# ChenyangLEI/All-In-One-Deflicker

Measured on NVIDIA H100. Metric: atlas_iters_per_sec, higher is better.
Workload: dtype fp32 (2-term fp16 split on wgmma, fp32 accumulate)

## Files before the change

### all-in-one-deflicker_b200/csrc/mlp_tc.cu

```cuda
#include <mutex>
#include <vector>

#include "tc_api.cuh"
#include "tc_ptx.cuh"
#include "loss_math.h"

namespace b200 {
using namespace ptx;

constexpr int TM = 128;
constexpr int HID = 256;
constexpr int ITEM_BYTES = 16384;
constexpr int CHUNK_BYTES = 4 * ITEM_BYTES;
constexpr float S_ACT = 16.0f;
constexpr float S_W = 256.0f;
constexpr int ATOM_BYTES = TM * 128;
constexpr int TILE_IMG_BYTES = 4 * ATOM_BYTES;
constexpr int PE_COLS = 40;

__host__ __device__ __forceinline__ int atom_off(int m, int k) {
  const int r = m & 7;
  return (m >> 3) * 1024 + r * 128 + (((k >> 3) ^ r) << 4) + ((k & 7) << 1);
}
__host__ __device__ __forceinline__ int item_off(int n, int k) {
  return (n >> 3) * 512 + (n & 7) * 64 + ((((k >> 3) ^ (n >> 1)) & 3) << 4) + ((k & 7) << 1);
}

struct NetImages {
  char* w_fwd; int64_t w_fwd_layer[B200_MAX_LAYERS]; int n_chunks_fwd[B200_MAX_LAYERS];
  char* w_bwd; int64_t w_bwd_layer[B200_MAX_LAYERS];
  char* act; char* dz;
  int64_t slot_stride, term_stride;
  char* pe; char* dzl; int64_t w64_term_stride;
  uint32_t* bits;
  int64_t rows;
};

struct TcLayout { NetImages map, atl; };

static char* align_tc(char* base) { return reinterpret_cast<char*>(round_up(reinterpret_cast<int64_t>(base), 1024)); }
static char* carve_tc(char*& p, int64_t bytes) { char* r = p; p += round_up(bytes, 1024); return r; }

static void plan_fwd_weights(const MlpShape& s, TcNet net, char*& p, NetImages* n) {
  const bool pe = tc_pe_first(net);
  int64_t off = 0;
  for (int l = 0; l < s.L; ++l) {
    int chunks = 0;
    const bool tc_layer = pe ? (l <= s.L - 2) : (l >= 1 && l <= s.L - 2);
    if (tc_layer) chunks = (l == 0 ? 0 : HID / 64) + ((l == 0 || s.skip[l]) && pe ? 1 : 0);
    n->n_chunks_fwd[l] = chunks;
    n->w_fwd_layer[l] = off;
    off += (int64_t)chunks * CHUNK_BYTES;
  }
  n->w_fwd = carve_tc(p, off);
}

static void plan_net(const MlpShape& s, int64_t rows, TcNet net, char*& p, NetImages* n) {
  const int64_t tiles = rows / TM;
  const bool pe = tc_pe_first(net);
  n->rows = rows;
  plan_fwd_weights(s, net, p, n);
  int64_t off = 0;
  for (int l = 0; l < s.L; ++l) {
    n->w_bwd_layer[l] = off;
    const bool used = l <= s.L - 2 && (pe || l >= 1);
    if (used) off += (int64_t)(HID / 64) * CHUNK_BYTES;
  }
  n->w_bwd = carve_tc(p, off);
  n->term_stride = tiles * TILE_IMG_BYTES;
  n->slot_stride = 2 * n->term_stride;
  n->act = carve_tc(p, (int64_t)(s.L - 1) * n->slot_stride);
  n->dz = carve_tc(p, (int64_t)(s.L - 1) * n->slot_stride);
  n->w64_term_stride = tiles * ATOM_BYTES;
  n->pe = pe ? carve_tc(p, 2 * n->w64_term_stride) : nullptr;
  n->dzl = carve_tc(p, 2 * n->w64_term_stride);
  n->bits = reinterpret_cast<uint32_t*>(carve_tc(p, (int64_t)(s.L - 1) * rows * 32));
}

int64_t tc_plan(const MlpShape& ms, const MlpShape& as, int64_t rows_map, int64_t rows_atlas, char* base,
                TcPlan* out) {
  char* p = align_tc(base);
  TcLayout lay{};
  plan_net(ms, rows_map, tc_net_of(ms), p, &lay.map);
  plan_net(as, rows_atlas, TcNet::Atlas, p, &lay.atl);
  if (out) { out->base = base; out->bytes = p - base; out->rows_map = rows_map; out->rows_atlas = rows_atlas; }
  return p - base;
}

static TcLayout layout_of(const TcStep& s) {
  char* p = align_tc(s.plan->base);
  TcLayout lay{};
  plan_net(*s.ms, s.plan->rows_map, tc_net_of(*s.ms), p, &lay.map);
  plan_net(*s.as, s.plan->rows_atlas, TcNet::Atlas, p, &lay.atl);
  return lay;
}

struct PrepJob {
  const float* W; int ldw;
  int n_rows, k0, k_cnt;
  int transpose;
  char* hi; char* lo;
};
constexpr int MAX_PREP_JOBS = 96;
struct PrepJobs { PrepJob j[MAX_PREP_JOBS]; int n; };

__global__ void tc_prep_kernel(const PrepJobs* __restrict__ jobs_ptr) {
  const PrepJob jb = jobs_ptr->j[blockIdx.x >> 2];
  for (int e = threadIdx.x; e < 64 * 8; e += blockDim.x) {
    const int row = (blockIdx.x & 3) * 64 + (e >> 3), c8 = (e & 7) * 8;
    float v[8];
#pragma unroll
    for (int q = 0; q < 8; ++q) {
      const int col = c8 + q;
      v[q] = 0.f;
      if (row < jb.n_rows && col < jb.k_cnt)
        v[q] = jb.transpose ? jb.W[(int64_t)(jb.k0 + col) * jb.ldw + row] : jb.W[(int64_t)row * jb.ldw + jb.k0 + col];
    }
    uint32_t h[4], l[4];
#pragma unroll
    for (int q = 0; q < 4; ++q) split2_f16(v[2 * q] * S_W, v[2 * q + 1] * S_W, h[q], l[q]);
    const int off = (c8 >> 5) * ITEM_BYTES + item_off(row, c8 & 31);
    *reinterpret_cast<uint4*>(jb.hi + off) = make_uint4(h[0], h[1], h[2], h[3]);
    *reinterpret_cast<uint4*>(jb.lo + off) = make_uint4(l[0], l[1], l[2], l[3]);
  }
}

template <int NST>
struct Pipe {
  uint64_t* full; uint64_t* empty; char* stage;
  uint32_t it;
  __device__ __forceinline__ int slot() const { return it % NST; }
  __device__ __forceinline__ uint32_t parity() const { return (it / NST) & 1; }
};

struct TileIter {
  int t0, tf, tb, total, cap_tiles, n_groups, gf, gb;
  __device__ __forceinline__ void init(int cap, int groups, const int* counters, int g_fwd, int g_bwd) {
    cap_tiles = cap / TM;
    n_groups = groups;
    gf = (counters && g_fwd < groups) ? g_fwd : -1;
    gb = (counters && g_bwd < groups) ? g_bwd : -1;
    t0 = counters ? min(cap_tiles, (counters[0] + TM - 1) / TM) : cap_tiles;
    tf = gf >= 0 ? min(cap_tiles, (counters[5] + TM - 1) / TM) : t0;
    tb = gb >= 0 ? min(cap_tiles, (counters[6] + TM - 1) / TM) : t0;
    total = t0 * (groups - (gf >= 0) - (gb >= 0)) + (gf >= 0 ? tf : 0) + (gb >= 0 ? tb : 0);
  }
  __device__ __forceinline__ int group_tiles(int g) const { return g == gf ? tf : (g == gb ? tb : t0); }
  __device__ __forceinline__ int global_tile(int t) const {
    for (int g = 0; g < n_groups; ++g) {
      const int n = group_tiles(g);
      if (t < n) return g * cap_tiles + t;
      t -= n;
    }
    return 0;
  }
};

template <int NST>
__device__ __forceinline__ void produce_items(Pipe<NST>& pp, const char* src, int n_items, uint32_t bytes = ITEM_BYTES) {
  for (int i = 0; i < n_items; ++i) {
    mbar_wait(&pp.empty[pp.slot()], pp.parity() ^ 1);
    mbar_expect_tx(&pp.full[pp.slot()], bytes);
    bulk_g2s(pp.stage + pp.slot() * ITEM_BYTES, src + (int64_t)i * ITEM_BYTES, bytes, &pp.full[pp.slot()]);
    ++pp.it;
  }
}

constexpr int CONSUMER_WGS = 2;
constexpr int CONSUMERS = CONSUMER_WGS * 128;
constexpr int TC_THREADS = CONSUMERS + 128;
constexpr int PRODUCER_REGS = 56, CONSUMER_REGS = 224;
constexpr int EMPTY_ARRIVALS = CONSUMER_WGS * 4;
constexpr int WG_ROW_BYTES = 8192;

struct Consumer {
  int g, w4, lane, q, tid;
  int m0;
  bool warp_leader, leader;
  __device__ __forceinline__ void init() {
    const int warp = warp_uniform();
    lane = threadIdx.x & 31; q = lane & 3;
    g = warp >> 2; w4 = warp & 3;
    tid = threadIdx.x & 127;
    m0 = 64 * g + 16 * w4 + (lane >> 2);
    warp_leader = lane == 0;
    leader = tid == 0;
  }
  __device__ __forceinline__ void sync() const { named_bar(1 + g, 128); }
};

__host__ __device__ __forceinline__ int tile_off(int m, int col) { return (col >> 6) * ATOM_BYTES + atom_off(m, col & 63); }

template <int NST, int NN>
__device__ __forceinline__ void consume_item(Pipe<NST>& pp, float (&acc)[NN / 2], uint32_t a_hi, uint32_t a_lo, bool with_lo,
                                             uint32_t& scale, int& pending, const Consumer& c) {
  mbar_wait(&pp.full[pp.slot()], pp.parity());
  const uint32_t sb = smem_u32(pp.stage + pp.slot() * ITEM_BYTES);
  wgmma_fence();
#pragma unroll
  for (int ks = 0; ks < 2; ++ks) {
    const uint64_t bd = make_desc_sw64(sb + ks * 32, 512);
    if constexpr (NN == 256) wgmma_n256<0, 0>(*reinterpret_cast<float(*)[128]>(&acc), make_desc(a_hi + ks * 32, 16, 1024), bd, scale);
    else wgmma_n64<0, 0>(*reinterpret_cast<float(*)[32]>(&acc), make_desc(a_hi + ks * 32, 16, 1024), bd, scale);
    scale = 1u;
    if (with_lo) {
      if constexpr (NN == 256) wgmma_n256<0, 0>(*reinterpret_cast<float(*)[128]>(&acc), make_desc(a_lo + ks * 32, 16, 1024), bd, 1u);
      else wgmma_n64<0, 0>(*reinterpret_cast<float(*)[32]>(&acc), make_desc(a_lo + ks * 32, 16, 1024), bd, 1u);
    }
  }
  wgmma_commit();
  wgmma_wait<1>();
  if (pending >= 0 && c.warp_leader) mbar_arrive(&pp.empty[pending]);
  pending = pp.slot();
  ++pp.it;
}
template <int NST, int NN>
__device__ __forceinline__ void consume_chunk(Pipe<NST>& pp, float (&acc)[NN / 2], uint32_t a_hi, uint32_t a_lo,
                                              uint32_t& scale, int& pending, const Consumer& c) {
  consume_item<NST, NN>(pp, acc, a_hi, a_lo, true, scale, pending, c);
  consume_item<NST, NN>(pp, acc, a_hi + 64, a_lo + 64, true, scale, pending, c);
  consume_item<NST, NN>(pp, acc, a_hi, a_lo, false, scale, pending, c);
  consume_item<NST, NN>(pp, acc, a_hi + 64, a_lo + 64, false, scale, pending, c);
}
template <int NST, int R>
__device__ __forceinline__ void finish_pass(Pipe<NST>& pp, float (&acc)[R], int& pending, const Consumer& c) {
  wgmma_wait<0>();
  acc_fence(acc);
  if (pending >= 0 && c.warp_leader) mbar_arrive(&pp.empty[pending]);
  pending = -1;
}

__device__ __forceinline__ void store_tile_rows(const Consumer& c, const char* a_tile, char* g_img, int64_t term_stride) {
  if (!c.leader) return;
#pragma unroll
  for (int term = 0; term < 2; ++term)
#pragma unroll
    for (int j = 0; j < 4; ++j)
      bulk_s2g(g_img + term * term_stride + j * ATOM_BYTES + c.g * WG_ROW_BYTES,
               a_tile + term * TILE_IMG_BYTES + j * ATOM_BYTES + c.g * WG_ROW_BYTES, WG_ROW_BYTES);
  bulk_commit();
}
__device__ __forceinline__ void a_tile_reusable(const Consumer& c) {
  if (c.leader) bulk_wait_read0();
  c.sync();
}
__device__ __forceinline__ void a_tile_written(const Consumer& c) {
  fence_proxy_async_smem();
  c.sync();
}

__device__ __forceinline__ uint32_t relu_flag(float v) { return (uint32_t)(-(int)__float_as_uint(v)) >> 31; }

__device__ __forceinline__ uint32_t piece_bits(uint32_t f0, uint32_t f1, int col) {
  const int i = col & 15;
  uint32_t b = (f0 << (15 - i)) | (f1 << (14 - i));
  return b;
}
__device__ __forceinline__ uint32_t quad_or(uint32_t b) {
  b |= __shfl_xor_sync(0xffffffffu, b, 1);
  b |= __shfl_xor_sync(0xffffffffu, b, 2);
  return b;
}
__device__ __forceinline__ float quad_sum(float v) {
  v += __shfl_xor_sync(0xffffffffu, v, 1);
  return v + __shfl_xor_sync(0xffffffffu, v, 2);
}

constexpr int SMEM_A = 2 * TILE_IMG_BYTES;
constexpr int SMEM_AUX = 2 * ATOM_BYTES;
constexpr int RSUM_B_BYTES = 64 * 16;
constexpr int BWD_ACC_FLOATS = 5 * 256 + 768;
constexpr int SMEM_BWD_CONST_FLOATS = CONSUMER_WGS * (RSUM_B_BYTES / 4 + BWD_ACC_FLOATS);
constexpr int SMEM_BARS = 256;
constexpr int SMEM_MAX = 227 * 1024;
template <bool ATLAS, bool BWD> struct KCfg {
  static constexpr int NST = BWD ? 5 : (ATLAS ? 4 : 6);
  static constexpr int SMEM = SMEM_A + NST * ITEM_BYTES + (ATLAS && !BWD ? SMEM_AUX : 0) +
                              (BWD ? SMEM_BWD_CONST_FLOATS * 4 : 0) + SMEM_BARS;
  static_assert(SMEM <= SMEM_MAX, "fused kernel exceeds the shared memory of one CTA");
  static_assert(SMEM + ITEM_BYTES > SMEM_MAX, "one more weight slot would fit");
  static_assert(2 * NST * 8 <= SMEM_BARS, "ring barriers exceed their shared-memory slot");
};

template <int NST>
struct SmemMap {
  char* a_tile; char* stage; char* aux; float* cst;
  uint64_t* full; uint64_t* empty;
  __device__ __forceinline__ void init(char* raw, int aux_bytes, int cst_floats) {
    char* p = raw;
    a_tile = p; p += SMEM_A;
    stage = p; p += NST * ITEM_BYTES;
    aux = p; p += aux_bytes;
    cst = reinterpret_cast<float*>(p); p += cst_floats * 4;
    full = reinterpret_cast<uint64_t*>(p);
    empty = full + NST;
  }
};

template <int NST>
__device__ __forceinline__ void setup_cta(SmemMap<NST>& sm) {
  if (threadIdx.x == 0) {
    if (smem_u32(sm.a_tile) & 1023u) __trap();
    for (int i = 0; i < NST; ++i) { mbar_init(&sm.full[i], 1); mbar_init(&sm.empty[i], EMPTY_ARRIVALS); }
    fence_barrier_init();
  }
  __syncthreads();
}
constexpr int BAR_CONSUMERS = 9;

struct FwdParams {
  const float* x;
  float* y;
  const float* params;
  int64_t w_off[B200_MAX_LAYERS], b_off[B200_MAX_LAYERS];
  NetImages img;
  int cap, n_groups; const int* n_valid;
  int g_fwd, g_bwd;
  float in_scale, in_shift;
  int store_images;
  int tanh_out;
  int pe_freqs;
};

template <bool ATLAS, int NL = (ATLAS ? 8 : 6), int VAR = 0>
__global__ void __launch_bounds__(TC_THREADS, 1) tc_fwd_kernel(const __grid_constant__ FwdParams P) {
  extern __shared__ __align__(1024) char smem_raw[];
  constexpr int NST = KCfg<ATLAS, false>::NST;
  SmemMap<NST> sm; sm.init(smem_raw, ATLAS ? SMEM_AUX : 0, 0);
  const int warp = warp_uniform(), lane = threadIdx.x & 31;
  constexpr int L = NL;
  constexpr int FIRST_TC = ATLAS ? 0 : 1;
  constexpr int LAST_TC = L - 2;
  constexpr bool PE3 = ATLAS && VAR > 0;
  constexpr bool SKIPS = ATLAS && !PE3;
  constexpr int OUT = ATLAS ? (PE3 ? VAR : 3) : 2;
  constexpr int KLAST = SKIPS ? 296 : 256;
  const int pe_cols = VAR == 1 ? 30 : 6 * P.pe_freqs;
  setup_cta(sm);
  TileIter ti; ti.init(P.cap, P.n_groups, P.n_valid, P.g_fwd, P.g_bwd);

  if (warp >= CONSUMER_WGS * 4) {
    setmaxnreg_dec<PRODUCER_REGS>();
    if (warp == CONSUMER_WGS * 4 && lane == 0) {
      Pipe<NST> pp{sm.full, sm.empty, sm.stage, 0};
      for (int t = blockIdx.x; t < ti.total; t += gridDim.x)
        for (int l = FIRST_TC; l <= LAST_TC; ++l) {
          const char* base = P.img.w_fwd + P.img.w_fwd_layer[l];
          if (ATLAS && l == 0) { produce_items(pp, base, 4); continue; }
          if (SKIPS && l == 4) produce_items(pp, base + (int64_t)4 * CHUNK_BYTES, 4);
          produce_items(pp, base, 16);
        }
    }
    return;
  }
  setmaxnreg_inc<CONSUMER_REGS>();
  Consumer c; c.init();
  Pipe<NST> pp{sm.full, sm.empty, sm.stage, 0};
  int pending = -1;
  const float inv_scale = 1.0f / S_W;
  uint16_t* bits16 = reinterpret_cast<uint16_t*>(P.img.bits);
  const float* wlast = P.params + P.w_off[L - 1];
  const uint32_t a_rows = smem_u32(sm.a_tile) + c.g * WG_ROW_BYTES;
  const uint32_t aux_rows = smem_u32(sm.aux) + c.g * WG_ROW_BYTES;
  float acc[128];
  for (int t = blockIdx.x; t < ti.total; t += gridDim.x) {
    const int gt = ti.global_tile(t);
    const int64_t row0 = (int64_t)gt * TM + c.m0;
    auto put = [&](int m, int col, float v0, float v1) {
      uint32_t h, lo;
      split2_packed(v0, v1, h, lo);
      const int off = tile_off(m, col);
      *reinterpret_cast<uint32_t*>(sm.a_tile + off) = h;
      *reinterpret_cast<uint32_t*>(sm.a_tile + TILE_IMG_BYTES + off) = lo;
    };
    uint32_t held0 = 0, held1 = 0;
    auto flags_out = [&](int slot, int i, int col, uint32_t b0, uint32_t b1) {
      if ((i & 1) == 0) { held0 = b0; held1 = b1; return; }
      b0 = quad_or(b0 | held0); b1 = quad_or(b1 | held1);
      if (P.store_images && c.q == 0) {
        bits16[((int64_t)slot * P.img.rows + row0) * 16 + (col >> 4)] = (uint16_t)b0;
        bits16[((int64_t)slot * P.img.rows + row0 + 8) * 16 + (col >> 4)] = (uint16_t)b1;
      }
    };
    if (ATLAS) {
      c.sync();
      for (int task = c.tid; task < 64 * 8; task += 128) {
        const int m = 64 * c.g + (task & 63), c8 = task >> 6;
        const int64_t row = (int64_t)gt * TM + m;
        float in[3] = {0.f, 0.f, 0.f};
        if (PE3) {
          const float4 xv = *reinterpret_cast<const float4*>(P.x + row * 4);
          in[0] = xv.x * P.in_scale + P.in_shift; in[1] = xv.y * P.in_scale + P.in_shift; in[2] = xv.z * P.in_scale + P.in_shift;
        } else {
          const float2 uv = *reinterpret_cast<const float2*>(P.x + row * 2);
          in[0] = uv.x * P.in_scale + P.in_shift; in[1] = uv.y * P.in_scale + P.in_shift;
        }
        float vals[8];
        if (PE3) {
#pragma unroll
          for (int i = 0; i < 8; ++i) {
            const int cc = c8 * 8 + i;
            float v = 0.f;
            if (cc < pe_cols) {
              const int k = cc / 6, r = cc - k * 6;
              const float a = in[r < 3 ? r : r - 3] * pe_freq(k);
              v = r < 3 ? sinf(a) : cosf(a);
            }
            vals[i] = v * S_ACT;
          }
        } else {
#pragma unroll
          for (int half_k = 0; half_k < 2; ++half_k) {
            const int k = c8 * 2 + half_k;
            float s0 = 0.f, s1 = 0.f, c0 = 0.f, c1 = 0.f;
            if (k < 10) {
              const float bk = pe_freq(k);
              const float a0 = in[0] * bk, a1 = in[1] * bk;
              s0 = sinf(a0); s1 = sinf(a1); c0 = cosf(a0); c1 = cosf(a1);
            }
            vals[half_k * 4 + 0] = s0 * S_ACT; vals[half_k * 4 + 1] = s1 * S_ACT;
            vals[half_k * 4 + 2] = c0 * S_ACT; vals[half_k * 4 + 3] = c1 * S_ACT;
          }
        }
        uint32_t h[4], lo[4];
#pragma unroll
        for (int q2 = 0; q2 < 4; ++q2) split2_f16(vals[2 * q2], vals[2 * q2 + 1], h[q2], lo[q2]);
        const int off = atom_off(m, c8 * 8);
        const uint4 vh = make_uint4(h[0], h[1], h[2], h[3]), vl = make_uint4(lo[0], lo[1], lo[2], lo[3]);
        *reinterpret_cast<uint4*>(sm.aux + off) = vh;
        *reinterpret_cast<uint4*>(sm.aux + ATOM_BYTES + off) = vl;
        if (P.store_images) {
          char* g_hi = P.img.pe + (int64_t)gt * ATOM_BYTES;
          *reinterpret_cast<uint4*>(g_hi + off) = vh;
          *reinterpret_cast<uint4*>(g_hi + P.img.w64_term_stride + off) = vl;
        }
      }
      fence_proxy_async_smem();
      c.sync();
    } else {
      const float4 x0 = *reinterpret_cast<const float4*>(P.x + row0 * 4);
      const float4 x1 = *reinterpret_cast<const float4*>(P.x + (row0 + 8) * 4);
      const float* W0 = P.params + P.w_off[0];
      const float* b0p = P.params + P.b_off[0];
      a_tile_reusable(c);
#pragma unroll
      for (int i = 0; i < 32; ++i) {
        const int col = 8 * i + 2 * c.q;
#pragma unroll
        for (int e = 0; e < 2; ++e) {
          const int n = col + e;
          const float bs = __ldg(b0p + n) * S_ACT;
          const float w0 = __ldg(W0 + n * 3) * S_ACT, w1 = __ldg(W0 + n * 3 + 1) * S_ACT, w2 = __ldg(W0 + n * 3 + 2) * S_ACT;
          acc[4 * i + e] = fmaxf(__fmaf_rn(x0.z, w2, __fmaf_rn(x0.y, w1, __fmaf_rn(x0.x, w0, bs))), 0.f);
          acc[4 * i + 2 + e] = fmaxf(__fmaf_rn(x1.z, w2, __fmaf_rn(x1.y, w1, __fmaf_rn(x1.x, w0, bs))), 0.f);
        }
        put(c.m0, col, acc[4 * i], acc[4 * i + 1]);
        put(c.m0 + 8, col, acc[4 * i + 2], acc[4 * i + 3]);
        flags_out(0, i, col, piece_bits(relu_flag(acc[4 * i]), relu_flag(acc[4 * i + 1]), col),
                  piece_bits(relu_flag(acc[4 * i + 2]), relu_flag(acc[4 * i + 3]), col));
      }
      a_tile_written(c);
      if (P.store_images) store_tile_rows(c, sm.a_tile, P.img.act + (int64_t)gt * TILE_IMG_BYTES, P.img.term_stride);
    }
    float outacc[2][OUT];
#pragma unroll
    for (int jj = 0; jj < OUT; ++jj) outacc[0][jj] = outacc[1][jj] = 0.f;
#pragma unroll 1
    for (int l = FIRST_TC; l <= LAST_TC; ++l) {
      uint32_t scale = 0u;
      if (ATLAS && (l == 0 || (SKIPS && l == 4)))
        consume_chunk<NST, 256>(pp, acc, aux_rows, aux_rows + ATOM_BYTES, scale, pending, c);
      if (l > 0)
        for (int kc = 0; kc < 4; ++kc)
          consume_chunk<NST, 256>(pp, acc, a_rows + kc * ATOM_BYTES, a_rows + TILE_IMG_BYTES + kc * ATOM_BYTES, scale,
                                  pending, c);
      finish_pass(pp, acc, pending, c);
      const bool last = (l == LAST_TC);
      const float* bias = P.params + P.b_off[l];
      a_tile_reusable(c);
#pragma unroll
      for (int i = 0; i < 32; ++i) {
        const int col = 8 * i + 2 * c.q;
        const float bs0 = __ldg(bias + col) * S_ACT, bs1 = __ldg(bias + col + 1) * S_ACT;
        float v[4];
        v[0] = fmaxf(__fmaf_rn(acc[4 * i], inv_scale, bs0), 0.f);
        v[1] = fmaxf(__fmaf_rn(acc[4 * i + 1], inv_scale, bs1), 0.f);
        v[2] = fmaxf(__fmaf_rn(acc[4 * i + 2], inv_scale, bs0), 0.f);
        v[3] = fmaxf(__fmaf_rn(acc[4 * i + 3], inv_scale, bs1), 0.f);
        if (last) {
#pragma unroll
          for (int jj = 0; jj < OUT; ++jj) {
            const float wa = __ldg(wlast + jj * KLAST + col) * (1.0f / S_ACT);
            const float wb = __ldg(wlast + jj * KLAST + col + 1) * (1.0f / S_ACT);
            outacc[0][jj] = fmaf(v[1], wb, fmaf(v[0], wa, outacc[0][jj]));
            outacc[1][jj] = fmaf(v[3], wb, fmaf(v[2], wa, outacc[1][jj]));
          }
        }
        if (!last || P.store_images) {
          put(c.m0, col, v[0], v[1]);
          put(c.m0 + 8, col, v[2], v[3]);
        }
        flags_out(l, i, col, piece_bits(relu_flag(v[0]), relu_flag(v[1]), col),
                  piece_bits(relu_flag(v[2]), relu_flag(v[3]), col));
      }
      a_tile_written(c);
      if (P.store_images)
        store_tile_rows(c, sm.a_tile, P.img.act + (int64_t)l * P.img.slot_stride + (int64_t)gt * TILE_IMG_BYTES,
                        P.img.term_stride);
    }
    if (SKIPS) {
#pragma unroll
      for (int rr = 0; rr < 2; ++rr) {
        const int m = c.m0 + 8 * rr;
        for (int k = c.q * 10; k < c.q * 10 + 10; ++k) {
          const int off = atom_off(m, k);
          const float pv = __half2float(*reinterpret_cast<const __half*>(sm.aux + off)) +
                           __half2float(*reinterpret_cast<const __half*>(sm.aux + ATOM_BYTES + off));
#pragma unroll
          for (int jj = 0; jj < OUT; ++jj)
            outacc[rr][jj] = fmaf(pv, __ldg(wlast + jj * KLAST + 256 + k) * (1.0f / S_ACT), outacc[rr][jj]);
        }
      }
    }
#pragma unroll
    for (int rr = 0; rr < 2; ++rr)
#pragma unroll
      for (int jj = 0; jj < OUT; ++jj) {
        const float o = quad_sum(outacc[rr][jj]) + __ldg(P.params + P.b_off[L - 1] + jj);
        if (c.q == 0) P.y[(row0 + 8 * rr) * OUT + jj] = P.tanh_out ? tanhf(o) : o;
      }
  }
  if (c.leader) bulk_wait_all0();
}

struct BwdParams {
  const float* dy;
  const float* y;
  const float* x;
  float* d_in;
  const float* params;
  float* grads;
  int64_t w_off[B200_MAX_LAYERS], b_off[B200_MAX_LAYERS];
  NetImages img;
  int cap, n_groups; const int* n_valid;
  int* gmax_bits;
  int g_fwd, g_bwd;
  float in_scale;
  int d_in_accumulate;
  int tanh_out;
};

__device__ __forceinline__ void grad_scales(const int* gmax_bits, bool mapping, float& s_g, float& inv_sg) {
  const float mx = __int_as_float(gmax_bits[mapping ? 1 : 0]);
  int e = 0;
  if (mx > 0.f && mx < 3.0e38f) frexpf(mx, &e);
  e = max(-60, min(60, e));
  s_g = ldexpf(1.0f, 13 - e);
  inv_sg = ldexpf(1.0f, e - 13);
}

template <bool ATLAS, int NL = (ATLAS ? 8 : 6), int VAR = 0>
__global__ void __launch_bounds__(TC_THREADS, 1) tc_bwd_kernel(const __grid_constant__ BwdParams P) {
  extern __shared__ __align__(1024) char smem_raw[];
  constexpr int NST = KCfg<ATLAS, true>::NST;
  SmemMap<NST> sm; sm.init(smem_raw, 0, SMEM_BWD_CONST_FLOATS);
  const int warp = warp_uniform(), lane = threadIdx.x & 31;
  constexpr int L = NL;
  constexpr bool PE3 = ATLAS && VAR > 0;
  constexpr bool SKIPS = ATLAS && !PE3;
  constexpr int OUT = ATLAS ? (PE3 ? VAR : 3) : 2;
  constexpr int KLAST = SKIPS ? 296 : 256;
  constexpr int LOW = 1;
  constexpr bool HAS_DPE = ATLAS && !PE3;
  constexpr bool MAPPING = OUT == 2;
  static_assert((L - 1) * 256 + (ATLAS ? 0 : 768) <= BWD_ACC_FLOATS, "gradient accumulators exceed their slice");
  char* rsum_b = reinterpret_cast<char*>(sm.cst);
  float* s_acc = sm.cst + CONSUMER_WGS * RSUM_B_BYTES / 4;
  for (int i = threadIdx.x; i < CONSUMER_WGS * BWD_ACC_FLOATS; i += blockDim.x) s_acc[i] = 0.f;
  setup_cta(sm);
  TileIter ti; ti.init(P.cap, P.n_groups, P.n_valid, P.g_fwd, P.g_bwd);
  float s_g, inv_sg;
  grad_scales(P.gmax_bits, MAPPING, s_g, inv_sg);

  if (warp >= CONSUMER_WGS * 4) {
    setmaxnreg_dec<PRODUCER_REGS>();
    if (warp == CONSUMER_WGS * 4 && lane == 0) {
      Pipe<NST> pp{sm.full, sm.empty, sm.stage, 0};
      for (int t = blockIdx.x; t < ti.total; t += gridDim.x)
        for (int l = L - 2; l >= (HAS_DPE ? 0 : LOW); --l)
          produce_items(pp, P.img.w_bwd + P.img.w_bwd_layer[l], 16, l == 0 ? 64 * 64 : ITEM_BYTES);
    }
    return;
  }
  setmaxnreg_inc<CONSUMER_REGS>();
  Consumer c; c.init();
  Pipe<NST> pp{sm.full, sm.empty, sm.stage, 0};
  int pending = -1;
  const float inv_dgrad = inv_sg * (1.0f / S_W);
  const uint16_t* bits16 = reinterpret_cast<const uint16_t*>(P.img.bits);
  const float* wlast = P.params + P.w_off[L - 1];
  const uint32_t a_rows = smem_u32(sm.a_tile) + c.g * WG_ROW_BYTES;
  const uint32_t b_rows = smem_u32(rsum_b) + c.g * RSUM_B_BYTES;
  float* g_acc = s_acc + c.g * BWD_ACC_FLOATS;
  float acc[128];
  auto row_sums = [&](int slot) {
    float (&red)[16] = *reinterpret_cast<float(*)[16]>(&acc);
    uint32_t a_base = a_rows, b_base = b_rows;
    asm volatile("" : "+r"(a_base), "+r"(b_base));
    const uint64_t ad = make_desc(a_base, ATOM_BYTES, 1024), bd = make_desc_rows16(b_base);
    wgmma_fence();
#pragma unroll
    for (int blk = 0; blk < 4; ++blk)
#pragma unroll
      for (int ks = 0; ks < 4; ++ks) {
        const uint64_t a = ad + ((blk * ATOM_BYTES + ks * 2048) >> 4), b = bd + ((ks * 256) >> 4);
        float (&d)[4] = *reinterpret_cast<float(*)[4]>(&red[4 * blk]);
        wgmma_n8<1, 1>(d, a, b, ks > 0 ? 1u : 0u);
        wgmma_n8<1, 1>(d, a + (TILE_IMG_BYTES >> 4), b, 1u);
      }
    wgmma_commit();
    wgmma_wait<0>();
    acc_fence(red);
    const bool w0 = !ATLAS && slot == 0;
    if (c.q == 0 || w0) {
#pragma unroll
      for (int blk = 0; blk < 4; ++blk)
#pragma unroll
        for (int rr = 0; rr < 2; ++rr) {
          const int n = 64 * blk + 16 * c.w4 + (c.lane >> 2) + 8 * rr;
          const float v = (red[4 * blk + 2 * rr] + red[4 * blk + 2 * rr + 1]) * inv_sg;
          if (c.q == 0) g_acc[slot * 256 + n] += v;
          else g_acc[(L - 1) * 256 + n * 3 + c.q - 1] += v * (1.0f / S_ACT);
        }
    }
  };
  auto put = [&](int m, int col, float v0, float v1) {
    uint32_t h, lo;
    split2_packed(__fmul_rn(v0, s_g), __fmul_rn(v1, s_g), h, lo);
    const int off = tile_off(m, col);
    *reinterpret_cast<uint32_t*>(sm.a_tile + off) = h;
    *reinterpret_cast<uint32_t*>(sm.a_tile + TILE_IMG_BYTES + off) = lo;
  };
  for (int t = blockIdx.x; t < ti.total; t += gridDim.x) {
    const int gt = ti.global_tile(t);
    const int64_t row0 = (int64_t)gt * TM + c.m0;
    float dzl[2][OUT];
#pragma unroll
    for (int rr = 0; rr < 2; ++rr)
#pragma unroll
      for (int jj = 0; jj < OUT; ++jj) {
        const int64_t row = row0 + 8 * rr;
        const float yv = P.y[row * OUT + jj];
        dzl[rr][jj] = P.dy[row * OUT + jj] * (P.tanh_out ? (1.0f - yv * yv) : 1.0f);
      }
#pragma unroll
    for (int jj = 0; jj < OUT; ++jj) {
      float sj = c.q == 0 ? dzl[0][jj] + dzl[1][jj] : 0.f;
#pragma unroll
      for (int o = 16; o > 0; o >>= 1) sj += __shfl_xor_sync(0xffffffffu, sj, o);
      if (lane == 0 && sj != 0.f) atomicAdd(P.grads + P.b_off[L - 1] + jj, sj);
    }
    if (c.q == 0) {
#pragma unroll
      for (int rr = 0; rr < 2; ++rr) {
        const int m = c.m0 + 8 * rr;
        uint32_t h0, l0, h1 = 0, l1 = 0;
        split2_f16(dzl[rr][0] * s_g, OUT > 1 ? dzl[rr][OUT > 1 ? 1 : 0] * s_g : 0.f, h0, l0);
        if (OUT == 3) split2_f16(dzl[rr][OUT - 1] * s_g, 0.f, h1, l1);
        char* g_hi = P.img.dzl + (int64_t)gt * ATOM_BYTES;
        char* g_lo = g_hi + P.img.w64_term_stride;
        const int r = m & 7;
        const int base = (m >> 3) * 1024 + r * 128;
#pragma unroll
        for (int c16 = 0; c16 < 8; ++c16) {
          const int off = base + ((c16 ^ r) << 4);
          *reinterpret_cast<uint4*>(g_hi + off) = c16 == 0 ? make_uint4(h0, h1, 0, 0) : make_uint4(0, 0, 0, 0);
          *reinterpret_cast<uint4*>(g_lo + off) = c16 == 0 ? make_uint4(l0, l1, 0, 0) : make_uint4(0, 0, 0, 0);
        }
      }
    }
    a_tile_reusable(c);
// ... 265 lines not shown
            bulk_g2s(dst + 16384, b, 4096, &full[slot]);
            bulk_g2s(dst + 32768, b + W.b_term, 4096, &full[slot]);
            continue;
          }
          for (int j = 0; j < 2; ++j) {
            const int64_t off = (int64_t)(2 * rank + j) * ATOM_BYTES;
            bulk_g2s(dst + j * 4096, a + off, 4096, &full[slot]);
            bulk_g2s(dst + 8192 + j * 4096, a + W.a_term + off, 4096, &full[slot]);
          }
          if (b_atoms == 4) {
            for (int j = 2 * rank; j < 2 * rank + 2; ++j) {
              bulk_g2s_multicast(dst + 16384 + j * 4096, b + (int64_t)j * ATOM_BYTES, 4096, &full[slot], 0x3);
              bulk_g2s_multicast(dst + 32768 + j * 4096, b + W.b_term + (int64_t)j * ATOM_BYTES, 4096, &full[slot], 0x3);
            }
          } else {
            bulk_g2s_multicast(dst + 16384 + rank * 16384, b + rank * W.b_term, 4096, &full[slot], 0x3);
          }
        }
      }
    }
  } else {
    setmaxnreg_inc<CONSUMER_REGS>();
    Consumer c; c.init();
    float s_gm, inv_gm, s_ga, inv_ga;
    grad_scales(gmax_bits, true, s_gm, inv_gm);
    grad_scales(gmax_bits, false, s_ga, inv_ga);
    const uint32_t peer_empty = mapa_shared(smem_u32(empty), rank ^ 1);
    uint32_t gs = 0;
    for (int it = cluster; it < n_items; it += n_clusters) {
      const WgradItem W = items->it[it];
      TileIter ti; ti.init(W.cap, W.n_groups, n_valid, W.g_fwd, W.g_bwd);
      int t_begin, t_end; unit_tiles(W, ti, t_begin, t_end);
      const int n_steps = (t_end - t_begin) * 4;
      if (n_steps == 0) continue;
      const float inv = (W.mapping ? inv_gm : inv_ga) * (1.0f / S_ACT);
      const int m0 = rank * 128 + c.g * 64;
      if (W.a_cols == 64) wgrad_unit<64, true>(W, n_steps / 2, 0, stage, full, empty, peer_empty, gs, c, inv);
      else if (W.b_cols == 256) wgrad_unit<256, false>(W, n_steps, m0, stage, full, empty, peer_empty, gs, c, inv);
      else wgrad_unit<64, false>(W, n_steps, m0, stage, full, empty, peer_empty, gs, c, inv);
    }
  }
  __syncthreads();
  if (threadIdx.x == 0 && blockIdx.x < 256) const_cast<WgradItems*>(items)->cycles[blockIdx.x] = clock64() - t_start;
  cluster_sync();
}

static int g_sm_count = 0;
static int sm_count() {
  if (!g_sm_count) {
    int dev = 0;
    cudaGetDevice(&dev);
    cudaDeviceGetAttribute(&g_sm_count, cudaDevAttrMultiProcessorCount, dev);
    if (g_sm_count <= 0) g_sm_count = 132;
  }
  return g_sm_count;
}

static int current_device() { int d = 0; cudaGetDevice(&d); return d; }

TcNet tc_net_of(const MlpShape& s) {
  if (s.hidden != HID) return TcNet::None;
  bool skips_4_7 = true, no_skips = true;
  for (int l = 1; l < s.L; ++l) {
    skips_4_7 = skips_4_7 && s.skip[l] == (l == 4 || l == 7);
    no_skips = no_skips && !s.skip[l];
  }
  if (s.L == 6 && s.pe == 0 && s.in_dim == 3 && s.out_dim == 2 && no_skips) return TcNet::Mapping6;
  if (s.L == 4 && s.pe == 0 && s.in_dim == 3 && s.out_dim == 2 && no_skips) return TcNet::Mapping4;
  if (s.L == 8 && s.pe == 10 && s.in_dim == 2 && s.out_dim == 3 && skips_4_7) return TcNet::Atlas;
  if (s.L == 8 && s.pe == 5 && s.in_dim == 3 && s.out_dim == 1 && no_skips) return TcNet::Alpha;
  const bool pe_chunk = s.pe >= 1 && s.pe <= 10;
  if (s.L == 6 && pe_chunk && s.in_dim == 3 && s.out_dim == 2 && no_skips) return TcNet::MappingPE6;
  if (s.L == 4 && pe_chunk && s.in_dim == 3 && s.out_dim == 2 && no_skips) return TcNet::MappingPE4;
  return TcNet::None;
}

struct NetKernels { void (*fwd)(FwdParams); void (*bwd)(BwdParams); int fwd_smem, bwd_smem; };
static const NetKernels g_kernels[] = {
    {tc_fwd_kernel<false, 6>, tc_bwd_kernel<false, 6>, KCfg<false, false>::SMEM, KCfg<false, true>::SMEM},
    {tc_fwd_kernel<false, 4>, tc_bwd_kernel<false, 4>, KCfg<false, false>::SMEM, KCfg<false, true>::SMEM},
    {tc_fwd_kernel<true, 8, 0>, tc_bwd_kernel<true, 8, 0>, KCfg<true, false>::SMEM, KCfg<true, true>::SMEM},
    {tc_fwd_kernel<true, 8, 1>, tc_bwd_kernel<true, 8, 1>, KCfg<true, false>::SMEM, KCfg<true, true>::SMEM},
    {tc_fwd_kernel<true, 6, 2>, tc_bwd_kernel<true, 6, 2>, KCfg<true, false>::SMEM, KCfg<true, true>::SMEM},
    {tc_fwd_kernel<true, 4, 2>, tc_bwd_kernel<true, 4, 2>, KCfg<true, false>::SMEM, KCfg<true, true>::SMEM},
};

static int g_wg_clusters[64];

static int ensure_attrs() {
  static bool done_dev[64] = {};
  int dev = 0;
  B200_CHECK_CUDA(cudaGetDevice(&dev));
  B200_REQUIRE(dev >= 0 && dev < 64, "device ordinal %d out of range", dev);
  bool& done = done_dev[dev];
  if (done) return B200_OK;
  for (const NetKernels& k : g_kernels) {
    B200_CHECK_CUDA(cudaFuncSetAttribute(k.fwd, cudaFuncAttributeMaxDynamicSharedMemorySize, k.fwd_smem));
    B200_CHECK_CUDA(cudaFuncSetAttribute(k.bwd, cudaFuncAttributeMaxDynamicSharedMemorySize, k.bwd_smem));
  }
  B200_CHECK_CUDA(cudaFuncSetAttribute(tc_wgrad_kernel, cudaFuncAttributeMaxDynamicSharedMemorySize, WG_SMEM));
  cudaLaunchConfig_t cfg = {};
  cfg.gridDim = dim3(WG_CLUSTER); cfg.blockDim = dim3(WG_THREADS); cfg.dynamicSmemBytes = WG_SMEM;
  B200_CHECK_CUDA(cudaOccupancyMaxActiveClusters(&g_wg_clusters[dev], tc_wgrad_kernel, &cfg));
  B200_REQUIRE(g_wg_clusters[dev] > 0, "the weight-gradient kernel's %d-CTA clusters do not fit on device %d", WG_CLUSTER, dev);
  done = true;
  return B200_OK;
}

static int launch_fwd(TcNet net, const FwdParams& P, int tiles, cudaStream_t st) {
  const NetKernels& k = g_kernels[(int)net - 1];
  k.fwd<<<min(sm_count(), tiles), TC_THREADS, k.fwd_smem, st>>>(P);
  B200_CHECK_LAUNCH();
  return B200_OK;
}

static int launch_bwd(TcNet net, const BwdParams& P, int tiles, cudaStream_t st) {
  const NetKernels& k = g_kernels[(int)net - 1];
  k.bwd<<<min(sm_count(), tiles), TC_THREADS, k.bwd_smem, st>>>(P);
  B200_CHECK_LAUNCH();
  return B200_OK;
}

static FwdParams fill_fwd(const MlpShape& sh, const NetImages& im, const float* x, float* y, const float* params, int cap,
                          int groups, const int* n_valid) {
  FwdParams P{};
  P.x = x; P.y = y; P.params = params; P.img = im; P.cap = cap; P.n_groups = groups; P.n_valid = n_valid;
  P.in_scale = 0.5f; P.in_shift = 0.5f; P.store_images = 1; P.tanh_out = 1; P.g_fwd = P.g_bwd = -1; P.pe_freqs = sh.pe;
  for (int l = 0; l < sh.L; ++l) { P.w_off[l] = sh.w_off[l]; P.b_off[l] = sh.b_off[l]; }
  return P;
}

static FwdParams fill_fwd_mapping(const MlpShape& sh, const NetImages& im, const float* x, float* y, const float* params,
                                  int cap, int groups, const int* n_valid) {
  FwdParams P = fill_fwd(sh, im, x, y, params, cap, groups, n_valid);
  P.in_scale = 1.0f; P.in_shift = 0.0f;
  return P;
}

static BwdParams fill_bwd(const MlpShape& sh, const NetImages& im, const float* dy, const float* y, const float* x,
                          float* d_in, const float* params, float* grads, int cap, int groups, const int* n_valid,
                          int* gmax_bits) {
  BwdParams P{};
  P.dy = dy; P.y = y; P.x = x; P.d_in = d_in; P.params = params; P.grads = grads; P.img = im;
  P.cap = cap; P.n_groups = groups; P.n_valid = n_valid; P.gmax_bits = gmax_bits;
  P.in_scale = 0.5f; P.d_in_accumulate = 1; P.tanh_out = 1; P.g_fwd = P.g_bwd = -1;
  for (int l = 0; l < sh.L; ++l) { P.w_off[l] = sh.w_off[l]; P.b_off[l] = sh.b_off[l]; }
  return P;
}

static void add_prep(PrepJobs& pj, const float* W, int ldw, int n_rows, int k0, int k_cnt, int transpose, char* dst) {
  PrepJob& j = pj.j[pj.n++];
  j.W = W; j.ldw = ldw; j.n_rows = n_rows; j.k0 = k0; j.k_cnt = k_cnt; j.transpose = transpose;
  j.hi = dst; j.lo = dst + 2 * ITEM_BYTES;
}

static void prep_jobs_for_net(PrepJobs& pj, const MlpShape& sh, const NetImages& im, const float* pp, TcNet net,
                              bool with_bwd) {
  const bool pe = tc_pe_first(net);
  for (int l = 0; l < sh.L; ++l) {
    char* dst = im.w_fwd + im.w_fwd_layer[l];
    if (im.n_chunks_fwd[l] == 0) continue;
    const float* W = pp + sh.w_off[l];
    int chunk = 0;
    if (l > 0) for (int kc = 0; kc < 4; ++kc) add_prep(pj, W, sh.K[l], 256, kc * 64, 64, 0, dst + (int64_t)(chunk++) * CHUNK_BYTES);
    if (pe && (l == 0 || sh.skip[l]))
      add_prep(pj, W, sh.K[l], 256, l == 0 ? 0 : 256, sh.enc, 0, dst + (int64_t)(chunk++) * CHUNK_BYTES);
  }
  if (!with_bwd) return;
  for (int l = 0; l < sh.L - 1; ++l) {
    if (l < 1 && !tc_net_has_dpe(net)) continue;
    char* dst = im.w_bwd + im.w_bwd_layer[l];
    const float* W = pp + sh.w_off[l];
    const int rows = (pe && l == 0) ? sh.enc : 256;
    for (int kc = 0; kc < 4; ++kc) add_prep(pj, W, sh.K[l], rows, kc * 64, 64, 1, dst + (int64_t)kc * CHUNK_BYTES);
  }
}

static double step_cost(int a_cols, int b_cols) {
  const int cols = a_cols + b_cols;
  return cols >= 512 ? 512.0 : (cols >= 320 ? 416.0 : 340.0);
}

struct WgProto { const char* a; int64_t a_term; int a_cols; const char* b; int64_t b_term; int b_cols; int transposed;
                 float* out; int ld; int n_rows, n_cols, groups; double bytes; int mapping; int g_fwd, g_bwd; };

static void protos_for_net(WgProto* protos, int& np, const MlpShape& sh, const NetImages& im, float* g, TcNet net,
                           int groups, int g_fwd = -1, int g_bwd = -1) {
  const bool pe = tc_pe_first(net);
  const int mapping = tc_net_is_mapping(net) ? 1 : 0;
  auto add = [&](const char* a, int64_t a_term, int a_cols, const char* b, int64_t b_term, int b_cols, float* out, int ld,
                 int n_rows, int n_cols, int transposed = 0) {
    protos[np++] = WgProto{a, a_term, a_cols, b, b_term, b_cols, transposed, out, ld, n_rows, n_cols, groups,
                           (double)groups * step_cost(a_cols, b_cols), mapping, g_fwd, g_bwd};
  };
  for (int l = 1; l <= sh.L - 2; ++l)
    add(im.dz + (int64_t)l * im.slot_stride, im.term_stride, 256, im.act + (int64_t)(l - 1) * im.slot_stride,
        im.term_stride, 256, g + sh.w_off[l], sh.K[l], 256, 256);
  add(im.act + (int64_t)(sh.L - 2) * im.slot_stride, im.term_stride, 256, im.dzl, im.w64_term_stride, 64,
      g + sh.w_off[sh.L - 1], sh.K[sh.L - 1], sh.out_dim, 256, 1);
  if (pe) {
    add(im.dz, im.term_stride, 256, im.pe, im.w64_term_stride, 64, g + sh.w_off[0], sh.K[0], 256, sh.enc);
    for (int l = 1; l <= sh.L - 2; ++l)
      if (sh.skip[l])
        add(im.dz + (int64_t)l * im.slot_stride, im.term_stride, 256, im.pe, im.w64_term_stride, 64, g + sh.w_off[l] + 256,
            sh.K[l], 256, sh.enc);
    if (sh.skip[sh.L - 1])
      add(im.dzl, im.w64_term_stride, 64, im.pe, im.w64_term_stride, 64, g + sh.w_off[sh.L - 1] + 256, sh.K[sh.L - 1],
          sh.out_dim, sh.enc);
  }
}

constexpr int WG_UNITS_PER_CLUSTER = 2;
static int wg_clusters() { return g_wg_clusters[current_device()]; }
static void apportion_items(WgradItems& wi, const WgProto* protos, int np, int cap) {
  double total_bytes = 0;
  for (int i = 0; i < np; ++i) total_bytes += protos[i].bytes;
  const int sms = wg_clusters() * WG_UNITS_PER_CLUSTER;
  int n_split[32], used = 0;
  double frac[32];
  for (int i = 0; i < np; ++i) {
    const double want = protos[i].bytes / total_bytes * sms;
    n_split[i] = (int)want < 1 ? 1 : (int)want;
    frac[i] = want - (int)want;
    used += n_split[i];
  }
  while (used < sms) {
    int best = 0;
    for (int i = 1; i < np; ++i) if (frac[i] > frac[best]) best = i;
    ++n_split[best]; frac[best] = -1.0; ++used;
  }
  while (used > sms) {
    int best = -1;
    for (int i = 0; i < np; ++i) if (n_split[i] > 1 && (best < 0 || n_split[i] > n_split[best])) best = i;
    if (best < 0) break;
    --n_split[best]; --used;
  }
  for (int i = 0; i < np; ++i) {
    for (int sp = 0; sp < n_split[i] && wi.n < MAX_WGRAD_ITEMS; ++sp) {
      WgradItem& it = wi.it[wi.n++];
      const WgProto& pr = protos[i];
      it.a_img = pr.a; it.a_term = pr.a_term; it.a_cols = pr.a_cols;
      it.b_img = pr.b; it.b_term = pr.b_term; it.b_cols = pr.b_cols; it.transposed = pr.transposed;
      it.out = pr.out; it.ld_out = pr.ld; it.n_rows = pr.n_rows; it.n_cols = pr.n_cols;
      it.cap = cap; it.n_groups = pr.groups; it.split = sp; it.n_split = n_split[i]; it.mapping = pr.mapping;
      it.g_fwd = pr.g_fwd; it.g_bwd = pr.g_bwd;
    }
  }
}

struct TabKey {
  int dev; const void* ws; TcNet net;
  int pe;
  bool step, with_bwd; int cap, groups, g_fwd, g_bwd;
  const void* params; const void* grads;
};
struct TcTables { TabKey key; PrepJobs* d_prep = nullptr; int n_prep = -1; WgradItems* d_wg = nullptr; int n_wg = -1; };
constexpr int MAX_TABLES = 4096;
static std::vector<TcTables*> g_tabs;
static std::mutex g_tabs_mutex;
static thread_local PrepJobs g_pj;
static thread_local WgradItems g_wi;

static TcTables* find_tables(const TabKey& k, bool add) {
  std::lock_guard<std::mutex> lock(g_tabs_mutex);
  for (TcTables* t : g_tabs) {
    TabKey& e = t->key;
    if (e.dev == k.dev && e.ws == k.ws && e.net == k.net && e.pe == k.pe && e.step == k.step && e.with_bwd == k.with_bwd &&
        e.cap == k.cap && e.groups == k.groups && e.g_fwd == k.g_fwd && e.g_bwd == k.g_bwd && e.params == k.params &&
        (!k.grads || !e.grads || e.grads == k.grads)) {
      if (!e.grads) e.grads = k.grads;
      return t;
    }
  }
  if (!add || (int)g_tabs.size() >= MAX_TABLES) return nullptr;
  g_tabs.push_back(new TcTables{k});
  return g_tabs.back();
}

template <class T> static int upload(const T& host, T** dst, bool own, cudaStream_t st) {
  cudaStreamCaptureStatus cs = cudaStreamCaptureStatusNone;
  cudaStreamIsCapturing(st, &cs);
  B200_REQUIRE(cs != cudaStreamCaptureStatusActive, "tensor-core job tables are uploaded by an eager call: run the same "
               "call once outside graph capture first (persistent workspaces only; the render is not capturable)");
  if (own) B200_CHECK_CUDA(cudaMalloc(dst, sizeof(T)));
  B200_CHECK_CUDA(cudaMemcpyAsync(*dst, &host, sizeof(T), cudaMemcpyHostToDevice, st));
  if (own) B200_CHECK_CUDA(cudaStreamSynchronize(st));
  return B200_OK;
}

static int step_g_fwd(const TcStep& s) { return (s.flow_groups && s.n_groups > 6) ? 5 : -1; }
static int step_g_bwd(const TcStep& s) { return (s.flow_groups && s.n_groups > 6) ? 6 : -1; }

static TabKey step_key(const TcStep& s) {
  return TabKey{current_device(), s.plan->base, s.y_atlas ? TcNet::Atlas : tc_net_of(*s.ms), s.ms->pe, true, true, s.cap,
                s.n_groups, step_g_fwd(s), step_g_bwd(s), s.params, s.grads};
}

static bool step_shapes_ok(const TcStep& s) {
  const TcNet m = tc_net_of(*s.ms);
  return (m == TcNet::Mapping6 || m == TcNet::MappingPE6) && tc_net_of(*s.as) == TcNet::Atlas;
}

struct SideStream { cudaStream_t stream = nullptr; cudaEvent_t fork = nullptr, join = nullptr; bool pending = false; };
static SideStream g_side[64];

int tc_begin_step(const TcStep& s, cudaStream_t st) {
  B200_PROPAGATE(ensure_attrs());
  TcTables* tab = find_tables(step_key(s), true);
  B200_REQUIRE(tab, "too many distinct tensor-core workspaces in one process (%d)", MAX_TABLES);
  if (tab->n_wg < 0) {
    B200_REQUIRE(step_shapes_ok(s), "tensor-core path is specialised to the two stage-1 networks (6-layer mapping, "
// ... 229 lines not shown
```

Before: 558.5.

## Stage pre-scaled forward biases and small weights in shared memory via bulk copy

```diff
diff --git a/all-in-one-deflicker_b200/csrc/mlp_tc.cu b/all-in-one-deflicker_b200/csrc/mlp_tc.cu
--- a/all-in-one-deflicker_b200/csrc/mlp_tc.cu
+++ b/all-in-one-deflicker_b200/csrc/mlp_tc.cu
@@ -26,8 +26,16 @@
   return (n >> 3) * 512 + (n & 7) * 64 + ((((k >> 3) ^ (n >> 1)) & 3) << 4) + ((k & 7) << 1);
 }
 
+struct FwdConsts { int w0, wl, bl, floats; };
+__host__ __device__ constexpr FwdConsts fwd_consts(int L, bool plain, int out, int k_last) {
+  const int w0 = (L - 1) * 256, wl = w0 + (plain ? 768 : 0), bl = wl + out * k_last;
+  return FwdConsts{w0, wl, bl, (bl + out + 3) / 4 * 4};
+}
+constexpr int FWD_CST_BYTES = 10752;
+
 struct NetImages {
   char* w_fwd; int64_t w_fwd_layer[B200_MAX_LAYERS]; int n_chunks_fwd[B200_MAX_LAYERS];
+  float* cst; int cst_floats;
   char* w_bwd; int64_t w_bwd_layer[B200_MAX_LAYERS];
   char* act; char* dz;
   int64_t slot_stride, term_stride;
@@ -53,6 +61,8 @@
     off += (int64_t)chunks * CHUNK_BYTES;
   }
   n->w_fwd = carve_tc(p, off);
+  n->cst_floats = fwd_consts(s.L, !pe, s.out_dim, s.K[s.L - 1]).floats;
+  n->cst = reinterpret_cast<float*>(carve_tc(p, (int64_t)n->cst_floats * 4));
 }
 
 static void plan_net(const MlpShape& s, int64_t rows, TcNet net, char*& p, NetImages* n) {
@@ -100,12 +110,18 @@
   int n_rows, k0, k_cnt;
   int transpose;
   char* hi; char* lo;
+  float* f32; float f32_scale;
 };
-constexpr int MAX_PREP_JOBS = 96;
+constexpr int MAX_PREP_JOBS = 128;
 struct PrepJobs { PrepJob j[MAX_PREP_JOBS]; int n; };
 
 __global__ void tc_prep_kernel(const PrepJobs* __restrict__ jobs_ptr) {
   const PrepJob jb = jobs_ptr->j[blockIdx.x >> 2];
+  if (jb.f32) {
+    for (int i = (blockIdx.x & 3) * blockDim.x + threadIdx.x; i < jb.n_rows; i += 4 * blockDim.x)
+      jb.f32[i] = jb.W[i] * jb.f32_scale;
+    return;
+  }
   for (int e = threadIdx.x; e < 64 * 8; e += blockDim.x) {
     const int row = (blockIdx.x & 3) * 64 + (e >> 3), c8 = (e & 7) * 8;
     float v[8];
@@ -274,12 +290,12 @@
 constexpr int SMEM_BARS = 256;
 constexpr int SMEM_MAX = 227 * 1024;
 template <bool ATLAS, bool BWD> struct KCfg {
-  static constexpr int NST = BWD ? 5 : (ATLAS ? 4 : 6);
+  static constexpr int NST = BWD ? 5 : (ATLAS ? 3 : 5);
   static constexpr int SMEM = SMEM_A + NST * ITEM_BYTES + (ATLAS && !BWD ? SMEM_AUX : 0) +
-                              (BWD ? SMEM_BWD_CONST_FLOATS * 4 : 0) + SMEM_BARS;
+                              (BWD ? SMEM_BWD_CONST_FLOATS * 4 : FWD_CST_BYTES) + SMEM_BARS;
   static_assert(SMEM <= SMEM_MAX, "fused kernel exceeds the shared memory of one CTA");
   static_assert(SMEM + ITEM_BYTES > SMEM_MAX, "one more weight slot would fit");
-  static_assert(2 * NST * 8 <= SMEM_BARS, "ring barriers exceed their shared-memory slot");
+  static_assert(2 * NST * 8 + 8 <= SMEM_BARS, "ring and constant barriers exceed their shared-memory slot");
 };
 
 template <int NST>
@@ -298,10 +314,11 @@
 };
 
 template <int NST>
-__device__ __forceinline__ void setup_cta(SmemMap<NST>& sm) {
+__device__ __forceinline__ void setup_cta(SmemMap<NST>& sm, bool cst_bar = false) {
   if (threadIdx.x == 0) {
     if (smem_u32(sm.a_tile) & 1023u) __trap();
     for (int i = 0; i < NST; ++i) { mbar_init(&sm.full[i], 1); mbar_init(&sm.empty[i], EMPTY_ARRIVALS); }
+    if (cst_bar) mbar_init(&sm.empty[NST], 1);
     fence_barrier_init();
   }
   __syncthreads();
@@ -326,7 +343,7 @@
 __global__ void __launch_bounds__(TC_THREADS, 1) tc_fwd_kernel(const __grid_constant__ FwdParams P) {
   extern __shared__ __align__(1024) char smem_raw[];
   constexpr int NST = KCfg<ATLAS, false>::NST;
-  SmemMap<NST> sm; sm.init(smem_raw, ATLAS ? SMEM_AUX : 0, 0);
+  SmemMap<NST> sm; sm.init(smem_raw, ATLAS ? SMEM_AUX : 0, FWD_CST_BYTES / 4);
   const int warp = warp_uniform(), lane = threadIdx.x & 31;
   constexpr int L = NL;
   constexpr int FIRST_TC = ATLAS ? 0 : 1;
@@ -335,13 +352,18 @@
   constexpr bool SKIPS = ATLAS && !PE3;
   constexpr int OUT = ATLAS ? (PE3 ? VAR : 3) : 2;
   constexpr int KLAST = SKIPS ? 296 : 256;
+  constexpr FwdConsts CST = fwd_consts(L, !ATLAS, OUT, KLAST);
+  static_assert(CST.floats * 4 <= FWD_CST_BYTES, "forward constants exceed their shared-memory slot");
+  uint64_t* cst_full = &sm.empty[NST];
   const int pe_cols = VAR == 1 ? 30 : 6 * P.pe_freqs;
-  setup_cta(sm);
+  setup_cta(sm, true);
   TileIter ti; ti.init(P.cap, P.n_groups, P.n_valid, P.g_fwd, P.g_bwd);
 
   if (warp >= CONSUMER_WGS * 4) {
     setmaxnreg_dec<PRODUCER_REGS>();
     if (warp == CONSUMER_WGS * 4 && lane == 0) {
+      mbar_expect_tx(cst_full, CST.floats * 4);
+      bulk_g2s(sm.cst, P.img.cst, CST.floats * 4, cst_full);
       Pipe<NST> pp{sm.full, sm.empty, sm.stage, 0};
       for (int t = blockIdx.x; t < ti.total; t += gridDim.x)
         for (int l = FIRST_TC; l <= LAST_TC; ++l) {
@@ -358,14 +380,15 @@
   Pipe<NST> pp{sm.full, sm.empty, sm.stage, 0};
   int pending = -1;
   const float inv_scale = 1.0f / S_W;
-  uint16_t* bits16 = reinterpret_cast<uint16_t*>(P.img.bits);
-  const float* wlast = P.params + P.w_off[L - 1];
+  const float* wlast = sm.cst + CST.wl;
   const uint32_t a_rows = smem_u32(sm.a_tile) + c.g * WG_ROW_BYTES;
   const uint32_t aux_rows = smem_u32(sm.aux) + c.g * WG_ROW_BYTES;
   float acc[128];
+  mbar_wait(cst_full, 0);
   for (int t = blockIdx.x; t < ti.total; t += gridDim.x) {
     const int gt = ti.global_tile(t);
     const int64_t row0 = (int64_t)gt * TM + c.m0;
+    uint16_t* bits_row = reinterpret_cast<uint16_t*>(P.img.bits) + row0 * 16;
     auto put = [&](int m, int col, float v0, float v1) {
       uint32_t h, lo;
       split2_packed(v0, v1, h, lo);
@@ -378,9 +401,17 @@
       if ((i & 1) == 0) { held0 = b0; held1 = b1; return; }
       b0 = quad_or(b0 | held0); b1 = quad_or(b1 | held1);
       if (P.store_images && c.q == 0) {
-        bits16[((int64_t)slot * P.img.rows + row0) * 16 + (col >> 4)] = (uint16_t)b0;
-        bits16[((int64_t)slot * P.img.rows + row0 + 8) * 16 + (col >> 4)] = (uint16_t)b1;
-      }
+        uint16_t* dst = bits_row + (int64_t)slot * P.img.rows * 16 + (col >> 4);
+        dst[0] = (uint16_t)b0;
+        dst[8 * 16] = (uint16_t)b1;
+      }
+    };
+    auto bias_relu = [&](const float* bias, int i, int col, float (&v)[4]) {
+      const float2 bs = *reinterpret_cast<const float2*>(bias + col);
+      v[0] = fmaxf(__fmaf_rn(acc[4 * i], inv_scale, bs.x), 0.f);
+      v[1] = fmaxf(__fmaf_rn(acc[4 * i + 1], inv_scale, bs.y), 0.f);
+      v[2] = fmaxf(__fmaf_rn(acc[4 * i + 2], inv_scale, bs.x), 0.f);
+      v[3] = fmaxf(__fmaf_rn(acc[4 * i + 3], inv_scale, bs.y), 0.f);
     };
     if (ATLAS) {
       c.sync();
@@ -440,19 +471,21 @@
     } else {
       const float4 x0 = *reinterpret_cast<const float4*>(P.x + row0 * 4);
       const float4 x1 = *reinterpret_cast<const float4*>(P.x + (row0 + 8) * 4);
-      const float* W0 = P.params + P.w_off[0];
-      const float* b0p = P.params + P.b_off[0];
+      const float* b0s = sm.cst;
+      const float* w0s = sm.cst + CST.w0;
       a_tile_reusable(c);
 #pragma unroll
       for (int i = 0; i < 32; ++i) {
         const int col = 8 * i + 2 * c.q;
+        const float2 bs = *reinterpret_cast<const float2*>(b0s + col);
+        const float2 wa = *reinterpret_cast<const float2*>(w0s + col * 3);
+        const float2 wb = *reinterpret_cast<const float2*>(w0s + col * 3 + 2);
+        const float2 wc = *reinterpret_cast<const float2*>(w0s + col * 3 + 4);
+        const float w[2][3] = {{wa.x, wa.y, wb.x}, {wb.y, wc.x, wc.y}}, b[2] = {bs.x, bs.y};
 #pragma unroll
         for (int e = 0; e < 2; ++e) {
-          const int n = col + e;
-          const float bs = __ldg(b0p + n) * S_ACT;
-          const float w0 = __ldg(W0 + n * 3) * S_ACT, w1 = __ldg(W0 + n * 3 + 1) * S_ACT, w2 = __ldg(W0 + n * 3 + 2) * S_ACT;
-          acc[4 * i + e] = fmaxf(__fmaf_rn(x0.z, w2, __fmaf_rn(x0.y, w1, __fmaf_rn(x0.x, w0, bs))), 0.f);
-          acc[4 * i + 2 + e] = fmaxf(__fmaf_rn(x1.z, w2, __fmaf_rn(x1.y, w1, __fmaf_rn(x1.x, w0, bs))), 0.f);
+          acc[4 * i + e] = fmaxf(__fmaf_rn(x0.z, w[e][2], __fmaf_rn(x0.y, w[e][1], __fmaf_rn(x0.x, w[e][0], b[e]))), 0.f);
+          acc[4 * i + 2 + e] = fmaxf(__fmaf_rn(x1.z, w[e][2], __fmaf_rn(x1.y, w[e][1], __fmaf_rn(x1.x, w[e][0], b[e]))), 0.f);
         }
         put(c.m0, col, acc[4 * i], acc[4 * i + 1]);
         put(c.m0 + 8, col, acc[4 * i + 2], acc[4 * i + 3]);
@@ -462,11 +495,7 @@
       a_tile_written(c);
       if (P.store_images) store_tile_rows(c, sm.a_tile, P.img.act + (int64_t)gt * TILE_IMG_BYTES, P.img.term_stride);
     }
-    float outacc[2][OUT];
-#pragma unroll
-    for (int jj = 0; jj < OUT; ++jj) outacc[0][jj] = outacc[1][jj] = 0.f;
-#pragma unroll 1
-    for (int l = FIRST_TC; l <= LAST_TC; ++l) {
+    auto mma_layer = [&](int l) {
       uint32_t scale = 0u;
       if (ATLAS && (l == 0 || (SKIPS && l == 4)))
         consume_chunk<NST, 256>(pp, acc, aux_rows, aux_rows + ATOM_BYTES, scale, pending, c);
@@ -475,25 +504,27 @@
           consume_chunk<NST, 256>(pp, acc, a_rows + kc * ATOM_BYTES, a_rows + TILE_IMG_BYTES + kc * ATOM_BYTES, scale,
                                   pending, c);
       finish_pass(pp, acc, pending, c);
-      const bool last = (l == LAST_TC);
-      const float* bias = P.params + P.b_off[l];
+    };
+    float outacc[2][OUT];
+#pragma unroll
+    for (int jj = 0; jj < OUT; ++jj) outacc[0][jj] = outacc[1][jj] = 0.f;
+#pragma unroll 1
+    for (int l = FIRST_TC; l <= LAST_TC; ++l) {
+      mma_layer(l);
+      const bool last = l == LAST_TC;
+      const float* bias = sm.cst + l * 256;
       a_tile_reusable(c);
 #pragma unroll
       for (int i = 0; i < 32; ++i) {
         const int col = 8 * i + 2 * c.q;
-        const float bs0 = __ldg(bias + col) * S_ACT, bs1 = __ldg(bias + col + 1) * S_ACT;
         float v[4];
-        v[0] = fmaxf(__fmaf_rn(acc[4 * i], inv_scale, bs0), 0.f);
-        v[1] = fmaxf(__fmaf_rn(acc[4 * i + 1], inv_scale, bs1), 0.f);
-        v[2] = fmaxf(__fmaf_rn(acc[4 * i + 2], inv_scale, bs0), 0.f);
-        v[3] = fmaxf(__fmaf_rn(acc[4 * i + 3], inv_scale, bs1), 0.f);
+        bias_relu(bias, i, col, v);
         if (last) {
 #pragma unroll
           for (int jj = 0; jj < OUT; ++jj) {
-            const float wa = __ldg(wlast + jj * KLAST + col) * (1.0f / S_ACT);
-            const float wb = __ldg(wlast + jj * KLAST + col + 1) * (1.0f / S_ACT);
-            outacc[0][jj] = fmaf(v[1], wb, fmaf(v[0], wa, outacc[0][jj]));
-            outacc[1][jj] = fmaf(v[3], wb, fmaf(v[2], wa, outacc[1][jj]));
+            const float2 w = *reinterpret_cast<const float2*>(wlast + jj * KLAST + col);
+            outacc[0][jj] = fmaf(v[1], w.y, fmaf(v[0], w.x, outacc[0][jj]));
+            outacc[1][jj] = fmaf(v[3], w.y, fmaf(v[2], w.x, outacc[1][jj]));
           }
         }
         if (!last || P.store_images) {
@@ -518,7 +549,7 @@
                            __half2float(*reinterpret_cast<const __half*>(sm.aux + ATOM_BYTES + off));
 #pragma unroll
           for (int jj = 0; jj < OUT; ++jj)
-            outacc[rr][jj] = fmaf(pv, __ldg(wlast + jj * KLAST + 256 + k) * (1.0f / S_ACT), outacc[rr][jj]);
+            outacc[rr][jj] = fmaf(pv, wlast[jj * KLAST + 256 + k], outacc[rr][jj]);
         }
       }
     }
@@ -526,7 +557,7 @@
     for (int rr = 0; rr < 2; ++rr)
 #pragma unroll
       for (int jj = 0; jj < OUT; ++jj) {
-        const float o = quad_sum(outacc[rr][jj]) + __ldg(P.params + P.b_off[L - 1] + jj);
+        const float o = quad_sum(outacc[rr][jj]) + sm.cst[CST.bl + jj];
         if (c.q == 0) P.y[(row0 + 8 * rr) * OUT + jj] = P.tanh_out ? tanhf(o) : o;
       }
   }
@@ -1098,11 +1129,22 @@
   PrepJob& j = pj.j[pj.n++];
   j.W = W; j.ldw = ldw; j.n_rows = n_rows; j.k0 = k0; j.k_cnt = k_cnt; j.transpose = transpose;
   j.hi = dst; j.lo = dst + 2 * ITEM_BYTES;
+  j.f32 = nullptr; j.f32_scale = 0.f;
+}
+static void add_const(PrepJobs& pj, const float* src, int n, float scale, float* dst) {
+  PrepJob& j = pj.j[pj.n++];
+  j = PrepJob{};
+  j.W = src; j.n_rows = n; j.f32 = dst; j.f32_scale = scale;
 }
 
 static void prep_jobs_for_net(PrepJobs& pj, const MlpShape& sh, const NetImages& im, const float* pp, TcNet net,
                               bool with_bwd) {
   const bool pe = tc_pe_first(net);
+  const FwdConsts fc = fwd_consts(sh.L, !pe, sh.out_dim, sh.K[sh.L - 1]);
+  for (int l = 0; l < sh.L - 1; ++l) add_const(pj, pp + sh.b_off[l], 256, S_ACT, im.cst + l * 256);
+  if (!pe) add_const(pj, pp + sh.w_off[0], 768, S_ACT, im.cst + fc.w0);
+  add_const(pj, pp + sh.w_off[sh.L - 1], sh.out_dim * sh.K[sh.L - 1], 1.0f / S_ACT, im.cst + fc.wl);
+  add_const(pj, pp + sh.b_off[sh.L - 1], sh.out_dim, 1.0f, im.cst + fc.bl);
   for (int l = 0; l < sh.L; ++l) {
     char* dst = im.w_fwd + im.w_fwd_layer[l];
     if (im.n_chunks_fwd[l] == 0) continue;
```

Measured after the change: 636.8, median of 6. 14.0% higher.
